# Accenture/AmpliGraph

Hardware: NVIDIA B200
Metric: training triples/sec (pos+eta negs) (higher is better)
Workload: dtype f32

## Files before the change

### ampligraph_b200/_lib.py

```python
import ctypes as C
import os
import subprocess

_HERE = os.path.dirname(os.path.abspath(__file__))
SO_PATH = os.environ.get("KGE_B200_LIB") or os.path.join(_HERE, "libkge_b200.so")
CSRC = os.path.join(_HERE, "csrc")
HEADER = os.path.join(os.path.dirname(_HERE), "include", "kge_b200.h")

KGE_OK, KGE_ERR_INVALID_ARGUMENT, KGE_ERR_CUDA, KGE_ERR_UNSUPPORTED = 0, 1, 2, 3
SCORING = {"TransE": 0, "DistMult": 1, "ComplEx": 2, "HolE": 3, "RotatE": 4}
LOSSES = {"pairwise": 0, "nll": 1, "absolute_margin": 2, "self_adversarial": 3, "multiclass_nll": 4}
REDUCTIONS = {"sum": 0, "mean": 1}
OPTIMIZERS = {"sgd": 0, "adam": 1, "adagrad": 2}
SIDES = {"s": 0, "o": 1}
STRATEGIES = {"worst": 0, "best": 1, "middle": 2}
STEP_FUSED, STEP_FORWARD_ONLY, STEP_BACKWARD_EXT = 0, 1, 2
RANK_MODES = {"auto": 0, "exact": 1}
INIT_KINDS = {"uniform": 0, "normal": 1, "truncated_normal": 2, "constant": 3}
ABI_VERSION = 2


class KgeConfig(C.Structure):
    _fields_ = [("struct_size", C.c_int32), ("scoring", C.c_int32), ("k", C.c_int32), ("eta", C.c_int32),
                ("n_ent", C.c_int64), ("n_rel", C.c_int64), ("loss", C.c_int32), ("reduction", C.c_int32),
                ("margin", C.c_float), ("alpha", C.c_float), ("device", C.c_int32), ("neg_group", C.c_int32),
                ("max_rel_size", C.c_int64), ("rank_mode", C.c_int32), ("rank_pair_cap", C.c_int32)]


class KgeOptimizerConfig(C.Structure):
    _fields_ = [("struct_size", C.c_int32), ("kind", C.c_int32), ("learning_rate", C.c_float),
                ("beta_1", C.c_float), ("beta_2", C.c_float), ("epsilon", C.c_float), ("momentum", C.c_float),
                ("initial_accumulator_value", C.c_float), ("reg_p", C.c_int32), ("reg_lambda", C.c_float),
                ("reg_p2", C.c_int32), ("reg_lambda2", C.c_float)]


class KgeShardMap(C.Structure):
    _fields_ = [("struct_size", C.c_int32), ("world", C.c_int32), ("rows_per_shard", C.c_int64),
                ("ent", C.c_void_p * 8), ("grad_ent", C.c_void_p * 8), ("stamp_ent", C.c_void_p * 8)]


_P = C.c_void_p
PROTOTYPES = {
    "kge_last_error": (C.c_char_p, []),
    "kge_abi_version": (C.c_int, []),
    "kge_create": (C.c_int, [C.POINTER(KgeConfig), C.POINTER(_P)]),
    "kge_destroy": (None, [_P]),
    "kge_internal_k": (C.c_int32, [_P]),
    "kge_half_stride": (C.c_int32, [_P]),
    "kge_row_stride": (C.c_int32, [_P]),
    "kge_pack_rows": (C.c_int, [_P, _P, _P, C.c_int64, _P]),
    "kge_unpack_rows": (C.c_int, [_P, _P, _P, C.c_int64, _P]),
    "kge_init_glorot_uniform": (C.c_int, [_P, _P, C.c_int64, C.c_uint64, _P]),
    "kge_init_table": (C.c_int, [_P, _P, C.c_int64, C.c_int32, C.c_float, C.c_float, C.c_uint64, _P]),
    "kge_score_triples": (C.c_int, [_P, _P, _P, _P, C.c_int64, _P, _P]),
    "kge_generate_corruptions": (C.c_int, [_P, _P, C.c_int64, C.c_uint64, C.c_uint64, _P, _P]),
    "kge_philox4x32_10": (None, [_P, _P, _P]),
    "kge_host_corruptions": (C.c_int, [_P, C.c_int64, C.c_int32, C.c_int64, C.c_uint64, C.c_uint64, _P]),
    "kge_train_step": (C.c_int, [_P, C.c_int32, _P, _P, _P, _P, _P, C.c_int64, _P, _P, C.c_uint64, C.c_uint64,
                                 _P, _P, _P, _P, _P, _P]),
    "kge_train_step_sharded": (C.c_int, [_P, C.c_int32, C.POINTER(KgeShardMap), _P, _P, _P, C.c_int64, _P, _P,
                                         C.c_uint64, C.c_uint64, _P, _P, _P, _P, _P, _P]),
    "kge_rank_sharded": (C.c_int, [_P, C.POINTER(KgeShardMap), C.c_int32, C.c_int32, C.c_int32, _P, _P, C.c_int64,
                                   _P, _P, C.c_int64, _P, _P, _P, C.c_int64, _P]),
    "kge_optimizer_step": (C.c_int, [_P, C.POINTER(KgeOptimizerConfig), C.c_int64, _P, _P, _P, _P, C.c_int64,
                                     _P, _P]),
    "kge_set_row_stamps": (C.c_int, [_P, _P, _P]),
    "kge_set_row_stash": (C.c_int, [_P, _P, C.c_int64]),
    "kge_set_hot_entities": (C.c_int, [_P, _P, C.c_int32]),
    "kge_rows_resident": (C.c_int, [_P]),
    "kge_step_stamp": (C.c_int32, [C.c_uint64]),
    "kge_optimizer_step_lazy": (C.c_int, [_P, C.POINTER(KgeOptimizerConfig), C.c_int64, _P, _P, _P, _P, C.c_int64, _P,
                                          C.c_int32, _P, _P]),
    "kge_optimizer_step_sharded": (C.c_int, [_P, C.POINTER(KgeOptimizerConfig), C.c_int64, C.c_int32, C.c_int32,
                                             C.POINTER(_P), C.POINTER(_P), _P, _P, C.c_int64, C.c_int64, _P, _P]),
    "kge_optimizer_step_exchange": (C.c_int, [_P, C.POINTER(KgeOptimizerConfig), C.POINTER(KgeOptimizerConfig), C.c_int64,
                                              C.c_int32, C.c_int32, C.POINTER(_P), C.POINTER(_P), _P, _P, _P, _P, _P,
                                              C.c_int64, C.c_int64, C.POINTER(_P), C.c_uint32, C.c_int32, _P, _P]),
    "kge_set_exchange_trace": (C.c_int, [_P, _P]),
    "kge_peer_barrier": (C.c_int, [_P, C.c_int32, C.c_int32, C.POINTER(_P), C.c_int32, C.c_uint32, _P]),
    "kge_rank": (C.c_int, [_P, C.c_int32, C.c_int32, _P, _P, _P, C.c_int64, _P, C.c_int64, C.c_int64, _P, _P,
                           C.c_int64, _P, _P, _P, C.c_int64, _P]),
    "kge_rank_finalize": (C.c_int, [_P, _P, C.c_int64, C.c_int32, _P, _P]),
    "kge_corruption_scores": (C.c_int, [_P, C.c_int32, _P, _P, _P, C.c_int64, _P, C.c_int64, C.c_int64, _P, _P,
                                        C.c_int64, _P]),
    "kge_rank_filter_probe": (C.c_int, [_P, C.c_int32, _P, _P, _P, C.c_int64, _P, C.c_int64, C.c_int64, _P, _P, _P,
                                        C.c_int64, _P]),
    "kge_rank_workspace_bytes": (C.c_int64, [_P, C.c_int64, C.c_int64]),
}

_lib = None


def build(verbose=False):
    cmd = ["make", "-C", CSRC, "-j8"]
    out = subprocess.run(cmd, stdout=subprocess.PIPE, stderr=subprocess.STDOUT, text=True)
    if verbose or out.returncode != 0:
        print(out.stdout)
    if out.returncode != 0:
        raise RuntimeError("building libkge_b200.so failed (see output above)")
    return SO_PATH


def load():
    global _lib
    if _lib is not None:
        return _lib
    if not os.path.exists(SO_PATH):
        raise RuntimeError(
            "ampligraph_b200: %s not found. Build it with `python -c 'import __graft_entry__ as g; g.build()'` "
            "or `make -C ampligraph_b200/csrc`. There is no CPU fallback for the CUDA path." % SO_PATH)
    lib = C.CDLL(SO_PATH)
    for name, (res, args) in PROTOTYPES.items():
        fn = getattr(lib, name)
        fn.restype = res
        fn.argtypes = args
    if lib.kge_abi_version() != ABI_VERSION:
        raise RuntimeError("libkge_b200.so ABI version %d, binding expects %d" % (lib.kge_abi_version(), ABI_VERSION))
    _lib = lib
    return lib


def check(rc):
# ... 19 lines not shown
```

### ampligraph_b200/csrc/kge_api.cu

```cuda
#include <stdarg.h>
#include <stdio.h>
#include <stdlib.h>
#include <string.h>

#include <new>

#include "kge_internal.h"

using namespace kge;

struct kge_handle {
    kge_config cfg;
    Layout L;
    int sm_count;
    int max_smem;
    float score_scale;
    float rot_div;
    float *rot;
    unsigned *done_counter;
    unsigned long long *exchange_trace;
    int nit, G, nbuf, warps, eta_pad, rows_bytes, region_bytes, wk, n_cb, slot_floats, resident;
    int res_warps, res_rows_bytes, res_region_bytes;
    int rot_warps, rot_G, rot_rows_bytes, rot_region_bytes;
    int *stamp_ent, *stamp_rel;
// ... 89 lines not shown
    Layout &L = h->L;
    L.model = cfg->scoring;
    L.k = cfg->k;
    L.halves = model_halves(cfg->scoring);
    L.kp = (cfg->k + 3) / 4 * 4;
    L.ld = L.halves * L.kp;
    L.K = L.halves * cfg->k;
    h->sm_count = prop.multiProcessorCount;
    h->max_smem = (int)prop.sharedMemPerBlockOptin;
    h->l2_bytes = prop.l2CacheSize;
    h->score_scale = (cfg->scoring == KGE_HOLE) ? hole_scale(L.K) : 1.f;
    h->rot_div = (cfg->scoring == KGE_ROTATE) ? rotate_divisor(L.K, cfg->max_rel_size > 0 ? cfg->max_rel_size : cfg->n_rel) : 1.f;

    const int nch = L.kp / 4;
    const int nit_raw = (nch + 31) / 32;
    h->nit = nit_raw <= 1 ? 1 : nit_raw <= 2 ? 2 : 4;
    h->wk = L.kp <= 512 ? L.kp : 512;
    h->n_cb = (L.kp + h->wk - 1) / h->wk;
    h->eta_pad = (cfg->eta + 3) / 4 * 4;
    const int row_bytes = L.halves * h->wk * 4, aux = 4 * h->eta_pad * 4 + 16;
    h->slot_floats = row_bytes / 4;
    int max_warps = KGE_TRAIN_THREADS(cfg->scoring, h->nit) / 32;
    int nbuf = 2;
    if (const char *ev = getenv("KGE_B200_TRAIN_WARPS")) { const int w = atoi(ev); if (w >= 1 && w < max_warps) max_warps = w; }
    if (const char *ev = getenv("KGE_B200_TRAIN_NBUF")) nbuf = atoi(ev) == 1 ? 1 : 2;
    int G = cfg->eta;
    bool res = h->n_cb == 1;
    if (cfg->neg_group > 0) {
        G = cfg->neg_group < cfg->eta ? cfg->neg_group : cfg->eta;
        res = res && G >= cfg->eta;
    } else {
        const long long full = (3 + (long long)cfg->eta) * row_bytes + aux;
        const int min_res = max_warps < KGE_MIN_RESIDENT_WARPS ? max_warps : KGE_MIN_RESIDENT_WARPS;
        if (!res || full * min_res > h->max_smem) {
            res = false;
            const int want = max_warps < KGE_TARGET_WARPS ? max_warps : KGE_TARGET_WARPS;
            while (G > 1 && (long long)((3 + nbuf * G) * (long long)row_bytes + aux) * want > h->max_smem) --G;
        }
    }
    h->resident = res ? 1 : 0;
    h->G = G;
    h->nbuf = nbuf;
    h->rows_bytes = (res ? 3 + G : 3 + nbuf * G) * row_bytes;
    h->region_bytes = h->rows_bytes + aux;
    int warps = h->max_smem / h->region_bytes;
    if (warps > max_warps) warps = max_warps;
    h->warps = warps;
    h->hot_ent[0] = h->hot_ent[1] = -1;

    h->res_warps = 0;
    if ((cfg->scoring == KGE_DISTMULT || cfg->scoring == KGE_COMPLEX || cfg->scoring == KGE_HOLE) && h->n_cb == 1 &&
        (h->nit <= 2 || cfg->scoring == KGE_DISTMULT) && cfg->eta <= 32 && cfg->neg_group <= 0) {
        const int res_aux = (3 * h->eta_pad * 4 + 8 + 15) / 16 * 16;
        h->res_rows_bytes = (2 + cfg->eta) * row_bytes;
        h->res_region_bytes = h->res_rows_bytes + res_aux;
        int rw = h->max_smem / h->res_region_bytes;
        if (rw > max_warps) rw = max_warps;
        int min_res = max_warps < KGE_MIN_RESIDENT_WARPS ? max_warps : KGE_MIN_RESIDENT_WARPS;
        if (h->nit == 4) min_res = KGE_MIN_RESIDENT_WARPS_WIDE;
        if (const char *ev = getenv("KGE_B200_RES_MIN_WARPS")) min_res = atoi(ev);
        if (rw >= min_res) h->res_warps = rw;
    }

    h->rot_warps = 0;
    if (cfg->scoring == KGE_ROTATE && h->n_cb == 1 && h->nit <= 2 && cfg->neg_group <= 0) {
        const int rot_aux = (4 * h->eta_pad * 4 + 16 + 15) / 16 * 16;
        const int rw = 8;
        const int cap = (h->max_smem / rw - rot_aux) / row_bytes;
        int rG = cap >= cfg->eta ? cfg->eta : cap / 2;
        if (const char *ev = getenv("KGE_B200_ROT_G")) {
            const int g = atoi(ev);
            if (g >= 1 && g <= cap / 2 && g < cfg->eta) rG = g;
        }
        if (rG >= 1) {
            h->rot_warps = rw;
            h->rot_G = rG;
            h->rot_rows_bytes = (rG >= cfg->eta ? rG : 2 * rG) * row_bytes;
            h->rot_region_bytes = h->rot_rows_bytes + rot_aux;
        }
    }

    if (cfg->scoring == KGE_ROTATE) {
        cudaError_t e2 = cudaMalloc(&h->rot, (size_t)cfg->n_rel * L.ld * sizeof(float));
        if (e2 != cudaSuccess) { delete h; return cuda_fail(e2, "cudaMalloc(rotation table)"); }
    }
    {
        cudaError_t e2 = cudaMalloc(&h->done_counter, 4 * sizeof(unsigned));
        if (e2 == cudaSuccess) e2 = cudaMemset(h->done_counter, 0, 4 * sizeof(unsigned));
        if (e2 != cudaSuccess) { if (h->rot) cudaFree(h->rot); delete h; return cuda_fail(e2, "cudaMalloc(counter)"); }
    }
    *out = h;
    return KGE_OK;
}

extern "C" void kge_destroy(kge_handle *h)
{
    if (!h) return;
    DeviceGuard guard_(h->cfg.device);
    if (h->rot) cudaFree(h->rot);
    if (h->done_counter) cudaFree(h->done_counter);
    delete h;
}

extern "C" int32_t kge_internal_k(const kge_handle *h) { return h ? h->L.K : 0; }
extern "C" int32_t kge_half_stride(const kge_handle *h) { return h ? h->L.kp : 0; }
extern "C" int32_t kge_row_stride(const kge_handle *h) { return h ? h->L.ld : 0; }

#define KGE_CHECK_HANDLE(h, fn)                                           \
    if (!(h)) return fail(KGE_ERR_INVALID_ARGUMENT, fn ": null handle"); \
    KGE_GUARD(h)

// ... 261 lines not shown
static RegParams reg_of(const kge_optimizer_config *opt)
{
    RegParams r;
    r.p = opt->reg_p; r.lambda = opt->reg_lambda; r.p2 = opt->reg_p2; r.lambda2 = opt->reg_lambda2;
    return r;
}
static void fill_optim(const kge_optimizer_config *opt, int64_t t, OptimParams &o)
{
    o.kind = opt->kind;
    o.lr = opt->learning_rate;
    o.beta1 = opt->beta_1;
    o.beta2 = opt->beta_2;
    o.eps = opt->epsilon;
    o.momentum = opt->momentum;
    o.reg = reg_of(opt);
    o.lr_t = (float)((double)opt->learning_rate * sqrt(1.0 - pow((double)opt->beta_2, (double)t)) /
                     (1.0 - pow((double)opt->beta_1, (double)t)));
}
static bool slots_ok(const kge_optimizer_config *opt, const float *s0, const float *s1)
{
    const bool need0 = opt->kind != KGE_OPT_SGD || opt->momentum != 0.f;
    const bool need1 = opt->kind == KGE_OPT_ADAM;
    return !((need0 && !s0) || (need1 && !s1));
}

extern "C" int kge_optimizer_step(kge_handle *h, const kge_optimizer_config *opt, int64_t t, float *table_dev,
                                  float *grad_dev, float *slot0_dev, float *slot1_dev, int64_t rows,
                                  double *reg_loss_dev, void *stream)
{
    KGE_CHECK_HANDLE(h, "kge_optimizer_step");
    if (int rc = check_optim(opt, "kge_optimizer_step")) return rc;
    if (rows < 0 || t < 1) return fail(KGE_ERR_INVALID_ARGUMENT, "kge_optimizer_step: rows >= 0 and t >= 1 required");
    if (rows == 0) return KGE_OK;
    if (!table_dev || !grad_dev) return fail(KGE_ERR_INVALID_ARGUMENT, "kge_optimizer_step: null table/grad");
    if (!slots_ok(opt, slot0_dev, slot1_dev))
        return fail(KGE_ERR_INVALID_ARGUMENT, "kge_optimizer_step: optimizer slot buffer missing");
    OptimParams o;
    fill_optim(opt, t, o);
    KGE_CUDA(launch_optimizer(o, table_dev, grad_dev, slot0_dev, slot1_dev, rows * (long long)h->L.ld, reg_loss_dev,
                              h->sm_count, (cudaStream_t)stream),
             "kge_optimizer_step");
    return KGE_OK;
}

extern "C" int kge_set_row_stamps(kge_handle *h, int32_t *ent_stamps_dev, int32_t *rel_stamps_dev)
{
    KGE_CHECK_HANDLE(h, "kge_set_row_stamps");
    h->stamp_ent = ent_stamps_dev;
    h->stamp_rel = rel_stamps_dev;
    return KGE_OK;
}

extern "C" int kge_rows_resident(const kge_handle *h) { return h ? (h->resident ? 1 : 0) : -1; }

extern "C" int kge_set_hot_entities(kge_handle *h, const int32_t *ids_host, int32_t n)
{
    KGE_CHECK_HANDLE(h, "kge_set_hot_entities");
    if (n < 0 || (n > 0 && !ids_host)) return fail(KGE_ERR_INVALID_ARGUMENT, "kge_set_hot_entities: bad arguments");
    h->hot_ent[0] = h->hot_ent[1] = -1;
    for (int i = 0; i < n && i < 2; ++i) {
        if (ids_host[i] < 0 || ids_host[i] >= h->cfg.n_ent) return fail(KGE_ERR_INVALID_ARGUMENT, "kge_set_hot_entities: id %d out of range", ids_host[i]);
        if (i == 1 && ids_host[1] == ids_host[0]) break;
        h->hot_ent[i] = ids_host[i];
    }
    return KGE_OK;
}

extern "C" int kge_set_row_stash(kge_handle *h, float *stash_dev, int64_t rows)
{
    KGE_CHECK_HANDLE(h, "kge_set_row_stash");
    if (rows < 0) return fail(KGE_ERR_INVALID_ARGUMENT, "kge_set_row_stash: rows < 0");
    h->stash = stash_dev;
    h->stash_rows = stash_dev ? rows : 0;
    return KGE_OK;
}

extern "C" int32_t kge_step_stamp(uint64_t step) { return (int32_t)(step & 0x3fffffffu) + 1; }

extern "C" int kge_optimizer_step_lazy(kge_handle *h, const kge_optimizer_config *opt, int64_t t, float *table_dev,
                                       float *grad_dev, float *slot0_dev, float *slot1_dev, int64_t rows,
                                       const int32_t *row_stamp_dev, int32_t stamp, double *reg_loss_dev, void *stream)
{
    KGE_CHECK_HANDLE(h, "kge_optimizer_step_lazy");
    if (int rc = check_optim(opt, "kge_optimizer_step_lazy")) return rc;
    if (rows < 0 || t < 1) return fail(KGE_ERR_INVALID_ARGUMENT, "kge_optimizer_step_lazy: rows >= 0 and t >= 1 required");
    if (rows == 0) return KGE_OK;
    if (!table_dev || !grad_dev || !row_stamp_dev) return fail(KGE_ERR_INVALID_ARGUMENT, "kge_optimizer_step_lazy: null pointer");
    if (!slots_ok(opt, slot0_dev, slot1_dev))
        return fail(KGE_ERR_INVALID_ARGUMENT, "kge_optimizer_step_lazy: optimizer slot buffer missing");
    OptimParams o;
    fill_optim(opt, t, o);
    KGE_CUDA(launch_optimizer_lazy(o, table_dev, grad_dev, slot0_dev, slot1_dev, rows, h->L.ld, (const int *)row_stamp_dev,
                                   stamp, reg_loss_dev, h->sm_count, (cudaStream_t)stream),
             "kge_optimizer_step_lazy");
    return KGE_OK;
}

static int check_world(int32_t world, int32_t rank, const char *fn)
{
    if (world < 1 || world > KGE_MAX_PEERS || rank < 0 || rank >= world)
        return fail(KGE_ERR_INVALID_ARGUMENT, "%s: world must be 1..%d and 0 <= rank < world", fn, KGE_MAX_PEERS);
    return KGE_OK;
}

extern "C" int kge_optimizer_step_sharded(kge_handle *h, const kge_optimizer_config *opt, int64_t t, int32_t world,
                                          int32_t rank, float *const *peer_tables, float *const *peer_grads,
// ... 265 lines not shown
```

### ampligraph_b200/csrc/kge_internal.h

```cpp
#pragma once
#include "kge_common.cuh"

#define KGE_TRAIN_THREADS(model, nit) ((nit) <= 1 ? 512 : (nit) == 2 ? ((model) == KGE_ROTATE ? 256 : 384) : 256)
#define KGE_MAX_PEERS 8
#define KGE_MIN_RESIDENT_WARPS 8
#define KGE_TARGET_WARPS 10
#define KGE_MIN_RESIDENT_WARPS_WIDE 6

namespace kge {

struct TrainParams {
    const float *ent;
    const float *rel;
    float *grad_ent;
    float *grad_rel;
    const int32_t *triples;
    long long B;
    const int32_t *neg_ent;
    const uint8_t *neg_keep;
    unsigned long long seed, step;
    unsigned n_ent;
    int model, eta, kp, ld, nch;
    int G;
    int nbuf;
    int wk, n_cb;
    int slot_floats;
    int resident;
    int eta_pad;
    int rows_bytes, region_bytes;
    int loss, reduction, mode;
    float margin, alpha, score_scale, inv_div;
    double *loss_out;
    float *scores_pos, *scores_neg;
    const float *dpos, *dneg;
    int shard_world, rows_per_shard;
    const float *ent_shard[KGE_MAX_PEERS];
    float *grad_ent_shard[KGE_MAX_PEERS];
    int stamp;
    int *stamp_ent, *stamp_rel;
    int *stamp_ent_shard[KGE_MAX_PEERS];
    int hot_ent[2];
    float *stash;
    unsigned *sched;
};

cudaError_t launch_train(const TrainParams &p, int nit, int sm_count, int threads, size_t smem, cudaStream_t st);
cudaError_t launch_train_res(const TrainParams &p, int nit, int sm_count, int threads, size_t smem, cudaStream_t st);
cudaError_t launch_train_rot(const TrainParams &p, int nit, int sm_count, int threads, size_t smem, cudaStream_t st);
cudaError_t launch_rotation_table(const float *rel, float *rot, long long n_rel, int kp, int ld, float div,
                                  cudaStream_t st);
cudaError_t launch_corruptions(const int32_t *triples, long long B, int eta, unsigned long long seed,
                               unsigned long long step, unsigned n_ent, int32_t *out, cudaStream_t st);

cudaError_t launch_score_triples(const Layout &L, int nit, const float *ent, const float *rel_or_rot,
                                 const int32_t *triples, long long n, float scale, float *out, int sm_count,
                                 cudaStream_t st);
// ... 83 lines not shown
```

### ampligraph_b200/csrc/kge_train_res.cu

```cuda
#include "kge_train_common.cuh"

namespace kge {

#ifndef KGE_HOT
#define KGE_HOT 1
#endif

template <int HALVES, int NIT, int THREADS>
__global__ void __launch_bounds__(THREADS) kge_train_res_kernel(const TrainParams p)
{
    extern __shared__ __align__(128) unsigned char smem_raw[];
    int warp = threadIdx.x >> 5, lane = threadIdx.x & 31;
    KGE_KEEP32(warp);
    KGE_KEEP32(lane);
    uint32_t rows_s = smem_u32(smem_raw) + (uint32_t)warp * (uint32_t)p.region_bytes;
    uint32_t sc_s = rows_s + (uint32_t)p.rows_bytes;
    uint32_t nid_s = sc_s + 4u * (uint32_t)p.eta_pad;
    uint32_t jor_s = nid_s + 4u * (uint32_t)p.eta_pad;
    uint32_t bar_s = jor_s + 4u * (uint32_t)p.eta_pad;
    KGE_KEEP32(rows_s); KGE_KEEP32(sc_s); KGE_KEEP32(nid_s); KGE_KEEP32(jor_s); KGE_KEEP32(bar_s);
    float *const sc = reinterpret_cast<float *>(smem_raw + (size_t)warp * p.region_bytes + p.rows_bytes);

    if (lane == 0) mbar_init_s(bar_s, 1);
    fence_mbar_init();
    fence_proxy_async_smem();
    __syncthreads();

    int ld = p.ld, eta = p.eta;
    const int nch = p.kp >> 2;
    uint32_t lwB = (uint32_t)p.slot_floats * 4u;
    uint32_t hsB = (uint32_t)p.kp * 4u;
    uint32_t row_bytes = (uint32_t)ld * 4u;
    KGE_KEEP32(ld); KGE_KEEP32(eta); KGE_KEEP32(lwB); KGE_KEEP32(hsB); KGE_KEEP32(row_bytes);
    uint32_t off[NIT];
    int live_i[NIT];
#pragma unroll
    for (int it = 0; it < NIT; ++it) {
        const int c = lane + 32 * it;
        live_i[it] = c < nch ? 1 : 0;
        off[it] = 16u * (uint32_t)min(c, nch - 1);
        KGE_KEEP32(off[it]);
        KGE_KEEP32(live_i[it]);
    }
    bool live[NIT];
#pragma unroll
    for (int it = 0; it < NIT; ++it) live[it] = live_i[it] != 0;
    float scale = p.score_scale;
    KGE_KEEPF(scale);
    unsigned lt = (1u << lane) - 1u;
    KGE_KEEP32(lt);
    float *grad_ent = p.grad_ent;
    KGE_KEEP64(grad_ent);
    const bool stamping = p.stamp_ent != nullptr && p.mode != KGE_STEP_FORWARD_ONLY;
    uint32_t phase = 0u;
    double loss_acc = 0.0;
    int hot0 = p.hot_ent[0], hot1 = KGE_HOT > 1 ? p.hot_ent[1] : -1;
    KGE_KEEP32(hot0); KGE_KEEP32(hot1);
    float4 H0r[NIT], H0i[NIT], H1r[NIT], H1i[NIT];
#pragma unroll
    for (int it = 0; it < NIT; ++it) H0r[it] = H0i[it] = H1r[it] = H1i[it] = f4zero();

    const long long n_warps = (long long)gridDim.x * (blockDim.x >> 5);
    float next_draw = 0.f;
    for (long long i = (long long)blockIdx.x * (blockDim.x >> 5) + warp; i < p.B;
         i = p.sched ? n_warps + (long long)(unsigned)__shfl_sync(0xffffffffu, next_draw, 0) : i + n_warps) {
        if (p.sched && lane == 0) next_draw = sched_draw(p.sched);
        int tv = 0;
        if (lane < 3) tv = __ldg(p.triples + 3 * i + lane);
        const int s_id = __shfl_sync(0xffffffffu, tv, 0), p_id = __shfl_sync(0xffffffffu, tv, 1), o_id = __shfl_sync(0xffffffffu, tv, 2);
        int keep = -1, repl = 0;
        if (lane < eta) {
            const unsigned long long r = (unsigned long long)lane * (unsigned long long)p.B + (unsigned long long)i;
            if (p.neg_ent) { repl = p.neg_ent[r]; keep = p.neg_keep[r] ? 1 : 0; }
            else draw_corruption(p.seed, p.step, r, p.n_ent, &keep, &repl);
        }
        const unsigned m0 = __ballot_sync(0xffffffffu, keep == 0), m1 = __ballot_sync(0xffffffffu, keep == 1);
        const int n0 = __popc(m0);
        if (lane < eta) {
            const int t = keep ? n0 + __popc(m1 & lt) : __popc(m0 & lt);
            sts_i(nid_s + 4u * (uint32_t)t, repl);
            sts_i(jor_s + 4u * (uint32_t)t, lane);
            if (stamping) p.stamp_ent[repl] = p.stamp;
        }
        if (stamping) {
            if (lane == 0) p.stamp_ent[s_id] = p.stamp;
            if (lane == 1) p.stamp_ent[o_id] = p.stamp;
            if (lane == 2 && p.stamp_rel) p.stamp_rel[p_id] = p.stamp;
        }
        __syncwarp();

        const int nrow = 2 + eta;
        if (lane == 0) mbar_expect_tx_s(bar_s, (uint32_t)nrow * row_bytes);
        __syncwarp();
        for (int r = lane; r < nrow; r += 32) {
            const int id = r == 0 ? s_id : r == 1 ? o_id : lds_i(nid_s + 4u * (uint32_t)(r - 2));
            bulk_load_s(rows_s + (uint32_t)r * lwB, p.ent + (size_t)id * ld, row_bytes, bar_s);
        }
        float4 pr[NIT], pi[NIT];
        {
            const char *prow = reinterpret_cast<const char *>(p.rel + (size_t)p_id * ld);
#pragma unroll
            for (int it = 0; it < NIT; ++it) {
                pr[it] = __ldg(reinterpret_cast<const float4 *>(prow + off[it]));
                if constexpr (HALVES == 2) pi[it] = __ldg(reinterpret_cast<const float4 *>(prow + off[it] + hsB));
                if (!live[it]) { pr[it] = f4zero(); pi[it] = f4zero(); }
            }
        }
        char *const gs_row = reinterpret_cast<char *>(grad_ent + (size_t)s_id * ld);
        char *const gp_row = reinterpret_cast<char *>(p.grad_rel + (size_t)p_id * ld);
        char *const go_row = reinterpret_cast<char *>(grad_ent + (size_t)o_id * ld);
        mbar_wait_s(bar_s, phase);
        phase ^= 1u;

        float4 Q0r[NIT], Q0i[NIT], Q1r[NIT], Q1i[NIT];
        float4 W0r[NIT], W0i[NIT], W1r[NIT], W1i[NIT];
        float P;
        {
            float4 acc = f4zero();
#pragma unroll
            for (int it = 0; it < NIT; ++it) {
                const uint32_t a = rows_s + off[it];
                if constexpr (HALVES == 2) {
                    const float4 sr = lds4(a), si = lds4(a + hsB);
                    const float4 orr = lds4(a + lwB), oi = lds4(a + lwB + hsB);
                    Q0r[it] = f4fma(pi[it], oi, pr[it] * orr);
                    Q0i[it] = pr[it] * oi - pi[it] * orr;
                    Q1r[it] = sr * pr[it] - si * pi[it];
                    Q1i[it] = f4fma(sr, pi[it], si * pr[it]);
                    acc = f4fma(sr, Q0r[it], acc);
                    acc = f4fma(si, Q0i[it], acc);
                    W0i[it] = W1i[it] = f4zero();
                } else {
                    const float4 vs = lds4(a), vo = lds4(a + lwB);
                    Q0r[it] = pr[it] * vo;
                    Q1r[it] = vs * pr[it];
                    acc = f4fma(vs, Q0r[it], acc);
                }
                W0r[it] = W1r[it] = f4zero();
            }
            P = warp_sum(f4hsum(acc));
        }

        auto score_side = [&](int lo, int hi, const float4(&qr)[NIT], const float4(&qi)[NIT]) {
            int t = lo;
            for (; hi - t >= 3; t += 4) {
                const uint32_t r0 = rows_s + (uint32_t)(2 + t) * lwB, r1 = r0 + lwB, r2 = r1 + lwB;
                const uint32_t r3 = (t + 3 < hi) ? r2 + lwB : r2;
                float4 a = f4zero(), b = f4zero(), c = f4zero(), d = f4zero();
#pragma unroll
                for (int it = 0; it < NIT; ++it) {
                    const uint32_t o = off[it];
                    a = f4fma(lds4(r0 + o), qr[it], a);
                    b = f4fma(lds4(r1 + o), qr[it], b);
                    c = f4fma(lds4(r2 + o), qr[it], c);
                    d = f4fma(lds4(r3 + o), qr[it], d);
                    if constexpr (HALVES == 2) {
                        a = f4fma(lds4(r0 + o + hsB), qi[it], a);
                        b = f4fma(lds4(r1 + o + hsB), qi[it], b);
                        c = f4fma(lds4(r2 + o + hsB), qi[it], c);
                        d = f4fma(lds4(r3 + o + hsB), qi[it], d);
                    }
                }
                const float v = warp_sum4t(f4hsum(a), f4hsum(b), f4hsum(c), f4hsum(d), lane);
                const int q = lane >> 3;
                if ((lane & 7) == 0 && t + q < hi) sts_f(sc_s + 4u * (uint32_t)(t + q), v);
            }
            if (t < hi) {
                const bool has_b = t + 1 < hi;
                const uint32_t ra = rows_s + (uint32_t)(2 + t) * lwB, rb = has_b ? ra + lwB : ra;
                float4 a = f4zero(), b = f4zero();
#pragma unroll
                for (int it = 0; it < NIT; ++it) {
                    const uint32_t o = off[it];
                    a = f4fma(lds4(ra + o), qr[it], a);
                    b = f4fma(lds4(rb + o), qr[it], b);
                    if constexpr (HALVES == 2) {
                        a = f4fma(lds4(ra + o + hsB), qi[it], a);
                        b = f4fma(lds4(rb + o + hsB), qi[it], b);
                    }
                }
                float pa = f4hsum(a), pb = f4hsum(b);
                warp_sum2(pa, pb);
                if (lane == 0) {
                    sts_f(sc_s + 4u * (uint32_t)t, pa);
                    if (has_b) sts_f(sc_s + 4u * (uint32_t)(t + 1), pb);
                }
            }
        };
        score_side(0, n0, Q0r, Q0i);
        score_side(n0, eta, Q1r, Q1i);
        __syncwarp();

        float dP;
        if (p.mode != KGE_STEP_BACKWARD_EXT) {
            if (scale != 1.f) {
                if (lane < eta) sc[lane] *= scale;
                __syncwarp();
            }
            if (p.scores_neg && lane < eta) p.scores_neg[(size_t)lds_i(jor_s + 4u * (uint32_t)lane) * p.B + i] = sc[lane];
            if (p.scores_pos && lane == 0) p.scores_pos[i] = scale * P;
            if (p.mode == KGE_STEP_FORWARD_ONLY) { __syncwarp(); continue; }
            const float li = loss_and_dscores(p, scale * P, sc, lane, &dP);
            if (lane == 0) loss_acc += (double)li;
        } else {
            if (lane < eta) sc[lane] = p.dneg[(size_t)lds_i(jor_s + 4u * (uint32_t)lane) * p.B + i];
            dP = p.dpos[i];
        }
        __syncwarp();

        auto red_row = [&](int id, float g, const float4(&qr)[NIT], const float4(&qi)[NIT]) {
            if (!live[0]) return;
            char *const g0 = reinterpret_cast<char *>(grad_ent + (size_t)id * ld) + off[0];
            char *const g1 = g0 + hsB;
#pragma unroll
            for (int it = 0; it < NIT; ++it) {
                if (!live[it]) break;
                red_add_v4(reinterpret_cast<float *>(g0 + 512 * it), g * qr[it]);
                if constexpr (HALVES == 2) red_add_v4(reinterpret_cast<float *>(g1 + 512 * it), g * qi[it]);
            }
        };
        auto grad_side = [&](int lo, int hi, const float4(&qr)[NIT], const float4(&qi)[NIT], float4(&Wr)[NIT], float4(&Wi)[NIT]) {
            for (int t = lo; t < hi; t += 2) {
                const bool has_b = t + 1 < hi;
                const uint32_t tb = (uint32_t)(has_b ? t + 1 : t);
                const uint32_t ra = rows_s + (uint32_t)(2 + t) * lwB, rb = rows_s + (2u + tb) * lwB;
                const float ga = scale * lds_f(sc_s + 4u * (uint32_t)t);
                const float gb = has_b ? scale * lds_f(sc_s + 4u * tb) : 0.f;
                const int ida = lds_i(nid_s + 4u * (uint32_t)t), idb = lds_i(nid_s + 4u * tb);
#pragma unroll
                for (int it = 0; it < NIT; ++it) {
                    const uint32_t o = off[it];
                    const float4 ar = lds4(ra + o), br = lds4(rb + o);
                    Wr[it] = f4fma(ga, ar, Wr[it]);
                    Wr[it] = f4fma(gb, br, Wr[it]);
                    if constexpr (HALVES == 2) {
                        const float4 ai = lds4(ra + o + hsB), bi = lds4(rb + o + hsB);
                        Wi[it] = f4fma(ga, ai, Wi[it]);
                        Wi[it] = f4fma(gb, bi, Wi[it]);
                    }
                }
                red_row(ida, ga, qr, qi);
                if (has_b) red_row(idb, gb, qr, qi);
            }
        };
        grad_side(0, n0, Q0r, Q0i, W0r, W0i);
        grad_side(n0, eta, Q1r, Q1i, W1r, W1i);

        {
            const float gP = scale * dP;
#pragma unroll
            for (int it = 0; it < NIT; ++it) {
                if (!live[it]) continue;
                const uint32_t o = off[it], a = rows_s + o;
                if constexpr (HALVES == 2) {
                    const float4 sr = lds4(a), si = lds4(a + hsB);
                    const float4 orr = lds4(a + lwB), oi = lds4(a + lwB + hsB);
                    const float4 Ur = f4fma(gP, sr, W0r[it]), Ui = f4fma(gP, si, W0i[it]);
                    const float4 Xr = f4fma(gP, orr, W1r[it]), Xi = f4fma(gP, oi, W1i[it]);
                    const float4 gsr = f4fma(pi[it], Xi, pr[it] * Xr), gsi = pr[it] * Xi - pi[it] * Xr;
                    const float4 gor = Ur * pr[it] - Ui * pi[it], goi = f4fma(Ur, pi[it], Ui * pr[it]);
                    if (s_id == hot0) { H0r[it] = H0r[it] + gsr; H0i[it] = H0i[it] + gsi; }
                    else if (KGE_HOT > 1 && s_id == hot1) { H1r[it] = H1r[it] + gsr; H1i[it] = H1i[it] + gsi; }
                    else { red4(gs_row, o, gsr); red4(gs_row, o + hsB, gsi); }
                    if (o_id == hot0) { H0r[it] = H0r[it] + gor; H0i[it] = H0i[it] + goi; }
                    else if (KGE_HOT > 1 && o_id == hot1) { H1r[it] = H1r[it] + gor; H1i[it] = H1i[it] + goi; }
                    else { red4(go_row, o, gor); red4(go_row, o + hsB, goi); }
                    red4(gp_row, o, f4fma(Ur, orr, Ui * oi) + f4fma(sr, W1r[it], si * W1i[it]));
                    red4(gp_row, o + hsB, (Ur * oi - Ui * orr) + (sr * W1i[it] - si * W1r[it]));
                } else {
                    const float4 vs = lds4(a), vo = lds4(a + lwB);
                    const float4 U = f4fma(gP, vs, W0r[it]), X = f4fma(gP, vo, W1r[it]);
                    const float4 gsr = pr[it] * X, gor = U * pr[it];
                    if (s_id == hot0) H0r[it] = H0r[it] + gsr;
                    else if (KGE_HOT > 1 && s_id == hot1) H1r[it] = H1r[it] + gsr;
                    else red4(gs_row, o, gsr);
                    if (o_id == hot0) H0r[it] = H0r[it] + gor;
                    else if (KGE_HOT > 1 && o_id == hot1) H1r[it] = H1r[it] + gor;
                    else red4(go_row, o, gor);
                    red4(gp_row, o, f4fma(U, vo, vs * W1r[it]));
                }
            }
        }
        __syncwarp();
    }
    sched_retire(p.sched, n_warps, lane);
    if (p.mode != KGE_STEP_FORWARD_ONLY) {
#pragma unroll
        for (int h = 0; h < KGE_HOT; ++h) {
            const int id = h ? hot1 : hot0;
            if (id < 0) continue;
            char *const row = reinterpret_cast<char *>(grad_ent + (size_t)id * ld);
#pragma unroll
            for (int it = 0; it < NIT; ++it) {
                if (!live[it]) continue;
                red4(row, off[it], h ? H1r[it] : H0r[it]);
                if constexpr (HALVES == 2) red4(row, off[it] + hsB, h ? H1i[it] : H0i[it]);
            }
        }
    }
    if (p.loss_out && p.mode == KGE_STEP_FUSED && lane == 0 && loss_acc != 0.0) atomicAdd(p.loss_out, loss_acc);
}

template <int HALVES, int NIT>
static cudaError_t launch_res(const TrainParams &p, int sm_count, int threads, size_t smem, cudaStream_t st)
{
    constexpr int THREADS = KGE_TRAIN_THREADS(KGE_COMPLEX, NIT);
    auto kern = kge_train_res_kernel<HALVES, NIT, THREADS>;
    cudaError_t e = cudaFuncSetAttribute(kern, cudaFuncAttributeMaxDynamicSharedMemorySize, (int)smem);
    if (e != cudaSuccess) return e;
    int occ = 0;
    e = cudaOccupancyMaxActiveBlocksPerMultiprocessor(&occ, kern, threads, smem);
    if (e != cudaSuccess) return e;
    if (occ < 1) return cudaErrorLaunchOutOfResources;
    const long long want = (p.B + (threads / 32) - 1) / (threads / 32), cap = (long long)occ * sm_count;
    kern<<<(int)(want < cap ? want : cap), threads, smem, st>>>(p);
    return cudaGetLastError();
}

cudaError_t launch_train_res(const TrainParams &p, int nit, int sm_count, int threads, size_t smem, cudaStream_t st)
{
    if (p.B == 0) return cudaSuccess;
    const bool two = p.model != KGE_DISTMULT;
    if (nit <= 1) return two ? launch_res<2, 1>(p, sm_count, threads, smem, st) : launch_res<1, 1>(p, sm_count, threads, smem, st);
    if (nit == 2) return two ? launch_res<2, 2>(p, sm_count, threads, smem, st) : launch_res<1, 2>(p, sm_count, threads, smem, st);
    if (two) return cudaErrorInvalidValue;
    return launch_res<1, 4>(p, sm_count, threads, smem, st);
}

}
```

### include/kge_b200.h

```cpp
#ifndef KGE_B200_H
#define KGE_B200_H

#include <stdint.h>

#ifdef __cplusplus
extern "C" {
#endif

#define KGE_B200_ABI_VERSION 2

typedef struct kge_handle kge_handle;

enum kge_status {
    KGE_OK = 0,
    KGE_ERR_INVALID_ARGUMENT = 1,
    KGE_ERR_CUDA = 2,
    KGE_ERR_UNSUPPORTED = 3
};

enum kge_scoring { KGE_TRANSE = 0, KGE_DISTMULT = 1, KGE_COMPLEX = 2, KGE_HOLE = 3, KGE_ROTATE = 4 };

enum kge_loss {
    KGE_LOSS_PAIRWISE = 0,
    KGE_LOSS_NLL = 1,
// ... 47 lines not shown
    int32_t reg_p;
    float reg_lambda;
    int32_t reg_p2;
    float reg_lambda2;
} kge_optimizer_config;

const char *kge_last_error(void);
int kge_abi_version(void);

int kge_create(const kge_config *cfg, kge_handle **out);
void kge_destroy(kge_handle *h);

int32_t kge_internal_k(const kge_handle *h);
int32_t kge_half_stride(const kge_handle *h);
int32_t kge_row_stride(const kge_handle *h);

int kge_pack_rows(kge_handle *h, const float *dense_dev, float *table_dev, int64_t rows, void *stream);
int kge_unpack_rows(kge_handle *h, const float *table_dev, float *dense_dev, int64_t rows, void *stream);

int kge_init_glorot_uniform(kge_handle *h, float *table_dev, int64_t rows, uint64_t seed, void *stream);
int kge_init_table(kge_handle *h, float *table_dev, int64_t rows, int32_t kind, float a, float b, uint64_t seed,
                   void *stream);

int kge_score_triples(kge_handle *h, const float *ent_dev, const float *rel_dev,
                      const int32_t *triples_dev , int64_t n, float *scores_dev ,
                      void *stream);

int kge_generate_corruptions(kge_handle *h, const int32_t *triples_dev, int64_t B, uint64_t seed,
                             uint64_t step, int32_t *corruptions_dev , void *stream);

void kge_philox4x32_10(const uint32_t ctr[4], const uint32_t key[2], uint32_t out[4]);
int kge_host_corruptions(const int32_t *triples_host , int64_t B, int32_t eta, int64_t n_ent,
                         uint64_t seed, uint64_t step, int32_t *corruptions_host );

int kge_train_step(kge_handle *h, int32_t mode, const float *ent_dev, const float *rel_dev,
                   float *grad_ent_dev, float *grad_rel_dev, const int32_t *triples_dev, int64_t B,
                   const int32_t *neg_ent_dev, const uint8_t *neg_keep_subj_dev, uint64_t seed,
                   uint64_t step, double *loss_dev, float *scores_pos_dev, float *scores_neg_dev,
                   const float *dpos_dev, const float *dneg_dev, void *stream);

typedef struct kge_shard_map {
    int32_t struct_size;
    int32_t world;
    int64_t rows_per_shard;
    const float *ent[8];
    float *grad_ent[8];
    int32_t *stamp_ent[8];
} kge_shard_map;

int kge_set_row_stash(kge_handle *h, float *stash_dev, int64_t rows);

int kge_set_hot_entities(kge_handle *h, const int32_t *ids_host, int32_t n);
int kge_rows_resident(const kge_handle *h);

int kge_train_step_sharded(kge_handle *h, int32_t mode, const kge_shard_map *map, const float *rel_dev,
                           float *grad_rel_dev, const int32_t *triples_dev, int64_t B,
                           const int32_t *neg_ent_dev, const uint8_t *neg_keep_subj_dev, uint64_t seed,
                           uint64_t step, double *loss_dev, float *scores_pos_dev, float *scores_neg_dev,
                           const float *dpos_dev, const float *dneg_dev, void *stream);

int kge_optimizer_step(kge_handle *h, const kge_optimizer_config *opt, int64_t t, float *table_dev,
                       float *grad_dev, float *slot0_dev, float *slot1_dev, int64_t rows,
                       double *reg_loss_dev, void *stream);

int kge_set_row_stamps(kge_handle *h, int32_t *ent_stamps_dev, int32_t *rel_stamps_dev);
int32_t kge_step_stamp(uint64_t step);
int kge_optimizer_step_lazy(kge_handle *h, const kge_optimizer_config *opt, int64_t t, float *table_dev,
                            float *grad_dev, float *slot0_dev, float *slot1_dev, int64_t rows,
                            const int32_t *row_stamp_dev, int32_t stamp, double *reg_loss_dev, void *stream);

int kge_optimizer_step_sharded(kge_handle *h, const kge_optimizer_config *opt, int64_t t, int32_t world,
                               int32_t rank, float *const *peer_tables, float *const *peer_grads,
                               float *slot0_shard_dev, float *slot1_shard_dev, int64_t row_begin,
                               int64_t row_end, double *reg_loss_dev, void *stream);

int kge_optimizer_step_exchange(kge_handle *h, const kge_optimizer_config *opt_ent,
                                const kge_optimizer_config *opt_rel, int64_t t, int32_t world, int32_t rank,
                                float *const *peer_tables, float *const *peer_grads, float *table_mc_dev,
                                const float *grads_mc_dev, float *zero_grads_dev,
                                float *slot0_shard_dev, float *slot1_shard_dev, int64_t row_begin,
                                int64_t row_end, uint32_t *const *peer_flags, uint32_t token, int32_t phases,
                                double *reg_loss_dev, void *stream);

int kge_set_exchange_trace(kge_handle *h, uint64_t *stamps_dev);

int kge_peer_barrier(kge_handle *h, int32_t world, int32_t rank, uint32_t *const *peer_flags, int32_t slot,
                     uint32_t token, void *stream);

int kge_rank(kge_handle *h, int32_t side, int32_t strategy, const float *ent_dev,
             const float *rel_dev, const int32_t *triples_dev, int64_t b,
             const int32_t *cand_ids_dev, int64_t cand_begin, int64_t n_cand,
             const int64_t *filt_off_dev, const int32_t *filt_idx_dev, int64_t n_filt,
             int32_t *ranks_dev, int32_t *counts_dev, void *workspace_dev, int64_t workspace_bytes,
             void *stream);

int kge_rank_sharded(kge_handle *h, const kge_shard_map *map, int32_t rank, int32_t side, int32_t strategy,
                     const float *rel_dev, const int32_t *triples_dev, int64_t b,
                     const int64_t *filt_off_dev, const int32_t *filt_idx_dev, int64_t n_filt,
                     int32_t *ranks_dev, int32_t *counts_dev, void *workspace_dev, int64_t workspace_bytes,
                     void *stream);

int kge_rank_finalize(kge_handle *h, const int32_t *counts_dev , int64_t b, int32_t strategy,
                      int32_t *ranks_dev, void *stream);

int kge_corruption_scores(kge_handle *h, int32_t side, const float *ent_dev, const float *rel_dev,
                          const int32_t *triples_dev, int64_t b, const int32_t *cand_ids_dev,
// ... 15 lines not shown
```

Baseline: 1.824 billion.

## Load s/o rows to registers, shrink smem region, add hot-free kernel variant

```diff
diff --git a/ampligraph_b200/_lib.py b/ampligraph_b200/_lib.py
--- a/ampligraph_b200/_lib.py
+++ b/ampligraph_b200/_lib.py
@@ -68,6 +68,7 @@
     "kge_set_row_stash": (C.c_int, [_P, _P, C.c_int64]),
     "kge_set_hot_entities": (C.c_int, [_P, _P, C.c_int32]),
     "kge_rows_resident": (C.c_int, [_P]),
+    "kge_train_fast_warps": (C.c_int, [_P]),
     "kge_step_stamp": (C.c_int32, [C.c_uint64]),
     "kge_optimizer_step_lazy": (C.c_int, [_P, C.POINTER(KgeOptimizerConfig), C.c_int64, _P, _P, _P, _P, C.c_int64, _P,
                                           C.c_int32, _P, _P]),
diff --git a/ampligraph_b200/csrc/kge_api.cu b/ampligraph_b200/csrc/kge_api.cu
--- a/ampligraph_b200/csrc/kge_api.cu
+++ b/ampligraph_b200/csrc/kge_api.cu
@@ -165,11 +165,13 @@
     if ((cfg->scoring == KGE_DISTMULT || cfg->scoring == KGE_COMPLEX || cfg->scoring == KGE_HOLE) && h->n_cb == 1 &&
         (h->nit <= 2 || cfg->scoring == KGE_DISTMULT) && cfg->eta <= 32 && cfg->neg_group <= 0) {
         const int res_aux = (3 * h->eta_pad * 4 + 8 + 15) / 16 * 16;
-        h->res_rows_bytes = (2 + cfg->eta) * row_bytes;
+        h->res_rows_bytes = cfg->eta * row_bytes;
         h->res_region_bytes = h->res_rows_bytes + res_aux;
+        int res_max = KGE_RES_THREADS(h->nit) / 32;
+        if (const char *ev = getenv("KGE_B200_TRAIN_WARPS")) { const int w = atoi(ev); if (w >= 1 && w < res_max) res_max = w; }
         int rw = h->max_smem / h->res_region_bytes;
-        if (rw > max_warps) rw = max_warps;
-        int min_res = max_warps < KGE_MIN_RESIDENT_WARPS ? max_warps : KGE_MIN_RESIDENT_WARPS;
+        if (rw > res_max) rw = res_max;
+        int min_res = res_max < KGE_MIN_RESIDENT_WARPS ? res_max : KGE_MIN_RESIDENT_WARPS;
         if (h->nit == 4) min_res = KGE_MIN_RESIDENT_WARPS_WIDE;
         if (const char *ev = getenv("KGE_B200_RES_MIN_WARPS")) min_res = atoi(ev);
         if (rw >= min_res) h->res_warps = rw;
@@ -537,6 +539,7 @@
 }
 
 extern "C" int kge_rows_resident(const kge_handle *h) { return h ? (h->resident ? 1 : 0) : -1; }
+extern "C" int kge_train_fast_warps(const kge_handle *h) { return h ? h->res_warps : -1; }
 
 extern "C" int kge_set_hot_entities(kge_handle *h, const int32_t *ids_host, int32_t n)
 {
diff --git a/ampligraph_b200/csrc/kge_internal.h b/ampligraph_b200/csrc/kge_internal.h
--- a/ampligraph_b200/csrc/kge_internal.h
+++ b/ampligraph_b200/csrc/kge_internal.h
@@ -2,6 +2,7 @@
 #include "kge_common.cuh"
 
 #define KGE_TRAIN_THREADS(model, nit) ((nit) <= 1 ? 512 : (nit) == 2 ? ((model) == KGE_ROTATE ? 256 : 384) : 256)
+#define KGE_RES_THREADS(nit) ((nit) <= 1 ? 512 : (nit) == 2 ? 448 : 256)
 #define KGE_MAX_PEERS 8
 #define KGE_MIN_RESIDENT_WARPS 8
 #define KGE_TARGET_WARPS 10
diff --git a/ampligraph_b200/csrc/kge_train_res.cu b/ampligraph_b200/csrc/kge_train_res.cu
--- a/ampligraph_b200/csrc/kge_train_res.cu
+++ b/ampligraph_b200/csrc/kge_train_res.cu
@@ -1,12 +1,19 @@
 #include "kge_train_common.cuh"
 
 namespace kge {
+
+__device__ __forceinline__ float4 ldg4_nc(const char *p)
+{
+    float4 v;
+    asm volatile("ld.global.nc.v4.f32 {%0, %1, %2, %3}, [%4];" : "=f"(v.x), "=f"(v.y), "=f"(v.z), "=f"(v.w) : "l"(p));
+    return v;
+}
 
 #ifndef KGE_HOT
 #define KGE_HOT 1
 #endif
 
-template <int HALVES, int NIT, int THREADS>
+template <int HALVES, int NIT, int THREADS, bool HOT>
 __global__ void __launch_bounds__(THREADS) kge_train_res_kernel(const TrainParams p)
 {
     extern __shared__ __align__(128) unsigned char smem_raw[];
@@ -89,28 +96,31 @@
         }
         __syncwarp();
 
-        const int nrow = 2 + eta;
-        if (lane == 0) mbar_expect_tx_s(bar_s, (uint32_t)nrow * row_bytes);
-        __syncwarp();
-        for (int r = lane; r < nrow; r += 32) {
-            const int id = r == 0 ? s_id : r == 1 ? o_id : lds_i(nid_s + 4u * (uint32_t)(r - 2));
-            bulk_load_s(rows_s + (uint32_t)r * lwB, p.ent + (size_t)id * ld, row_bytes, bar_s);
-        }
+        if (lane == 0) mbar_expect_tx_s(bar_s, (uint32_t)eta * row_bytes);
+        __syncwarp();
+        if (lane < eta) bulk_load_s(rows_s + (uint32_t)lane * lwB, p.ent + (size_t)lds_i(nid_s + 4u * (uint32_t)lane) * ld, row_bytes, bar_s);
         float4 pr[NIT], pi[NIT];
+        float4 sr[NIT], si[NIT], orr[NIT], oi[NIT];
         {
+            const char *const s_src = reinterpret_cast<const char *>(p.ent + (size_t)s_id * ld);
+            const char *const o_src = reinterpret_cast<const char *>(p.ent + (size_t)o_id * ld);
             const char *prow = reinterpret_cast<const char *>(p.rel + (size_t)p_id * ld);
 #pragma unroll
             for (int it = 0; it < NIT; ++it) {
+                sr[it] = __ldg(reinterpret_cast<const float4 *>(s_src + off[it]));
+                orr[it] = __ldg(reinterpret_cast<const float4 *>(o_src + off[it]));
                 pr[it] = __ldg(reinterpret_cast<const float4 *>(prow + off[it]));
-                if constexpr (HALVES == 2) pi[it] = __ldg(reinterpret_cast<const float4 *>(prow + off[it] + hsB));
+                if constexpr (HALVES == 2) {
+                    si[it] = __ldg(reinterpret_cast<const float4 *>(s_src + off[it] + hsB));
+                    oi[it] = __ldg(reinterpret_cast<const float4 *>(o_src + off[it] + hsB));
+                    pi[it] = __ldg(reinterpret_cast<const float4 *>(prow + off[it] + hsB));
+                }
                 if (!live[it]) { pr[it] = f4zero(); pi[it] = f4zero(); }
             }
         }
         char *const gs_row = reinterpret_cast<char *>(grad_ent + (size_t)s_id * ld);
         char *const gp_row = reinterpret_cast<char *>(p.grad_rel + (size_t)p_id * ld);
         char *const go_row = reinterpret_cast<char *>(grad_ent + (size_t)o_id * ld);
-        mbar_wait_s(bar_s, phase);
-        phase ^= 1u;
 
         float4 Q0r[NIT], Q0i[NIT], Q1r[NIT], Q1i[NIT];
         float4 W0r[NIT], W0i[NIT], W1r[NIT], W1i[NIT];
@@ -119,32 +129,30 @@
             float4 acc = f4zero();
 #pragma unroll
             for (int it = 0; it < NIT; ++it) {
-                const uint32_t a = rows_s + off[it];
-                if constexpr (HALVES == 2) {
-                    const float4 sr = lds4(a), si = lds4(a + hsB);
-                    const float4 orr = lds4(a + lwB), oi = lds4(a + lwB + hsB);
-                    Q0r[it] = f4fma(pi[it], oi, pr[it] * orr);
-                    Q0i[it] = pr[it] * oi - pi[it] * orr;
-                    Q1r[it] = sr * pr[it] - si * pi[it];
-                    Q1i[it] = f4fma(sr, pi[it], si * pr[it]);
-                    acc = f4fma(sr, Q0r[it], acc);
-                    acc = f4fma(si, Q0i[it], acc);
+                if constexpr (HALVES == 2) {
+                    Q0r[it] = f4fma(pi[it], oi[it], pr[it] * orr[it]);
+                    Q0i[it] = pr[it] * oi[it] - pi[it] * orr[it];
+                    Q1r[it] = sr[it] * pr[it] - si[it] * pi[it];
+                    Q1i[it] = f4fma(sr[it], pi[it], si[it] * pr[it]);
+                    acc = f4fma(sr[it], Q0r[it], acc);
+                    acc = f4fma(si[it], Q0i[it], acc);
                     W0i[it] = W1i[it] = f4zero();
                 } else {
-                    const float4 vs = lds4(a), vo = lds4(a + lwB);
-                    Q0r[it] = pr[it] * vo;
-                    Q1r[it] = vs * pr[it];
-                    acc = f4fma(vs, Q0r[it], acc);
+                    Q0r[it] = pr[it] * orr[it];
+                    Q1r[it] = sr[it] * pr[it];
+                    acc = f4fma(sr[it], Q0r[it], acc);
                 }
                 W0r[it] = W1r[it] = f4zero();
             }
             P = warp_sum(f4hsum(acc));
         }
+        mbar_wait_s(bar_s, phase);
+        phase ^= 1u;
 
         auto score_side = [&](int lo, int hi, const float4(&qr)[NIT], const float4(&qi)[NIT]) {
             int t = lo;
             for (; hi - t >= 3; t += 4) {
-                const uint32_t r0 = rows_s + (uint32_t)(2 + t) * lwB, r1 = r0 + lwB, r2 = r1 + lwB;
+                const uint32_t r0 = rows_s + (uint32_t)t * lwB, r1 = r0 + lwB, r2 = r1 + lwB;
                 const uint32_t r3 = (t + 3 < hi) ? r2 + lwB : r2;
                 float4 a = f4zero(), b = f4zero(), c = f4zero(), d = f4zero();
 #pragma unroll
@@ -167,7 +175,7 @@
             }
             if (t < hi) {
                 const bool has_b = t + 1 < hi;
-                const uint32_t ra = rows_s + (uint32_t)(2 + t) * lwB, rb = has_b ? ra + lwB : ra;
+                const uint32_t ra = rows_s + (uint32_t)t * lwB, rb = has_b ? ra + lwB : ra;
                 float4 a = f4zero(), b = f4zero();
 #pragma unroll
                 for (int it = 0; it < NIT; ++it) {
@@ -223,7 +231,7 @@
             for (int t = lo; t < hi; t += 2) {
                 const bool has_b = t + 1 < hi;
                 const uint32_t tb = (uint32_t)(has_b ? t + 1 : t);
-                const uint32_t ra = rows_s + (uint32_t)(2 + t) * lwB, rb = rows_s + (2u + tb) * lwB;
+                const uint32_t ra = rows_s + (uint32_t)t * lwB, rb = rows_s + tb * lwB;
                 const float ga = scale * lds_f(sc_s + 4u * (uint32_t)t);
                 const float gb = has_b ? scale * lds_f(sc_s + 4u * tb) : 0.f;
                 const int ida = lds_i(nid_s + 4u * (uint32_t)t), idb = lds_i(nid_s + 4u * tb);
@@ -243,39 +251,64 @@
                 if (has_b) red_row(idb, gb, qr, qi);
             }
         };
+#if KGE_RES_PREFETCH
+        {
+            const long long ent_off = reinterpret_cast<const char *>(p.ent) - reinterpret_cast<const char *>(grad_ent);
+#pragma unroll
+            for (int it = 0; it < NIT; ++it) {
+                asm volatile("prefetch.global.L1 [%0];" ::"l"(gs_row + ent_off + off[it]));
+                asm volatile("prefetch.global.L1 [%0];" ::"l"(go_row + ent_off + off[it]));
+                if constexpr (HALVES == 2) {
+                    asm volatile("prefetch.global.L1 [%0];" ::"l"(gs_row + ent_off + off[it] + hsB));
+                    asm volatile("prefetch.global.L1 [%0];" ::"l"(go_row + ent_off + off[it] + hsB));
+                }
+            }
+        }
+#endif
         grad_side(0, n0, Q0r, Q0i, W0r, W0i);
         grad_side(n0, eta, Q1r, Q1i, W1r, W1i);
 
         {
             const float gP = scale * dP;
+            const long long ent_off = reinterpret_cast<const char *>(p.ent) - reinterpret_cast<const char *>(grad_ent);
+            const char *const s_src = gs_row + ent_off, *const o_src = go_row + ent_off;
+            float4 vsr[NIT], vsi[NIT], vor[NIT], voi[NIT];
+#pragma unroll
+            for (int it = 0; it < NIT; ++it) {
+                vsr[it] = ldg4_nc(s_src + off[it]);
+                vor[it] = ldg4_nc(o_src + off[it]);
+                if constexpr (HALVES == 2) {
+                    vsi[it] = ldg4_nc(s_src + off[it] + hsB);
+                    voi[it] = ldg4_nc(o_src + off[it] + hsB);
+                }
+            }
 #pragma unroll
             for (int it = 0; it < NIT; ++it) {
                 if (!live[it]) continue;
-                const uint32_t o = off[it], a = rows_s + o;
-                if constexpr (HALVES == 2) {
-                    const float4 sr = lds4(a), si = lds4(a + hsB);
-                    const float4 orr = lds4(a + lwB), oi = lds4(a + lwB + hsB);
+                const uint32_t o = off[it];
+                if constexpr (HALVES == 2) {
+                    const float4 sr = vsr[it], si = vsi[it], orr = vor[it], oi = voi[it];
                     const float4 Ur = f4fma(gP, sr, W0r[it]), Ui = f4fma(gP, si, W0i[it]);
                     const float4 Xr = f4fma(gP, orr, W1r[it]), Xi = f4fma(gP, oi, W1i[it]);
                     const float4 gsr = f4fma(pi[it], Xi, pr[it] * Xr), gsi = pr[it] * Xi - pi[it] * Xr;
                     const float4 gor = Ur * pr[it] - Ui * pi[it], goi = f4fma(Ur, pi[it], Ui * pr[it]);
-                    if (s_id == hot0) { H0r[it] = H0r[it] + gsr; H0i[it] = H0i[it] + gsi; }
-                    else if (KGE_HOT > 1 && s_id == hot1) { H1r[it] = H1r[it] + gsr; H1i[it] = H1i[it] + gsi; }
+                    if (HOT && s_id == hot0) { H0r[it] = H0r[it] + gsr; H0i[it] = H0i[it] + gsi; }
+                    else if (HOT && KGE_HOT > 1 && s_id == hot1) { H1r[it] = H1r[it] + gsr; H1i[it] = H1i[it] + gsi; }
                     else { red4(gs_row, o, gsr); red4(gs_row, o + hsB, gsi); }
-                    if (o_id == hot0) { H0r[it] = H0r[it] + gor; H0i[it] = H0i[it] + goi; }
-                    else if (KGE_HOT > 1 && o_id == hot1) { H1r[it] = H1r[it] + gor; H1i[it] = H1i[it] + goi; }
+                    if (HOT && o_id == hot0) { H0r[it] = H0r[it] + gor; H0i[it] = H0i[it] + goi; }
+                    else if (HOT && KGE_HOT > 1 && o_id == hot1) { H1r[it] = H1r[it] + gor; H1i[it] = H1i[it] + goi; }
                     else { red4(go_row, o, gor); red4(go_row, o + hsB, goi); }
                     red4(gp_row, o, f4fma(Ur, orr, Ui * oi) + f4fma(sr, W1r[it], si * W1i[it]));
                     red4(gp_row, o + hsB, (Ur * oi - Ui * orr) + (sr * W1i[it] - si * W1r[it]));
                 } else {
-                    const float4 vs = lds4(a), vo = lds4(a + lwB);
+                    const float4 vs = vsr[it], vo = vor[it];
                     const float4 U = f4fma(gP, vs, W0r[it]), X = f4fma(gP, vo, W1r[it]);
                     const float4 gsr = pr[it] * X, gor = U * pr[it];
-                    if (s_id == hot0) H0r[it] = H0r[it] + gsr;
-                    else if (KGE_HOT > 1 && s_id == hot1) H1r[it] = H1r[it] + gsr;
+                    if (HOT && s_id == hot0) H0r[it] = H0r[it] + gsr;
+                    else if (HOT && KGE_HOT > 1 && s_id == hot1) H1r[it] = H1r[it] + gsr;
                     else red4(gs_row, o, gsr);
-                    if (o_id == hot0) H0r[it] = H0r[it] + gor;
-                    else if (KGE_HOT > 1 && o_id == hot1) H1r[it] = H1r[it] + gor;
+                    if (HOT && o_id == hot0) H0r[it] = H0r[it] + gor;
+                    else if (HOT && KGE_HOT > 1 && o_id == hot1) H1r[it] = H1r[it] + gor;
                     else red4(go_row, o, gor);
                     red4(gp_row, o, f4fma(U, vo, vs * W1r[it]));
                 }
@@ -284,7 +317,7 @@
         __syncwarp();
     }
     sched_retire(p.sched, n_warps, lane);
-    if (p.mode != KGE_STEP_FORWARD_ONLY) {
+    if (HOT && p.mode != KGE_STEP_FORWARD_ONLY) {
 #pragma unroll
         for (int h = 0; h < KGE_HOT; ++h) {
             const int id = h ? hot1 : hot0;
@@ -304,8 +337,9 @@
 template <int HALVES, int NIT>
 static cudaError_t launch_res(const TrainParams &p, int sm_count, int threads, size_t smem, cudaStream_t st)
 {
-    constexpr int THREADS = KGE_TRAIN_THREADS(KGE_COMPLEX, NIT);
-    auto kern = kge_train_res_kernel<HALVES, NIT, THREADS>;
+    constexpr int THREADS = KGE_RES_THREADS(NIT);
+    const bool hot = p.hot_ent[0] >= 0 || (KGE_HOT > 1 && p.hot_ent[1] >= 0);
+    auto kern = hot ? kge_train_res_kernel<HALVES, NIT, THREADS, true> : kge_train_res_kernel<HALVES, NIT, THREADS, false>;
     cudaError_t e = cudaFuncSetAttribute(kern, cudaFuncAttributeMaxDynamicSharedMemorySize, (int)smem);
     if (e != cudaSuccess) return e;
     int occ = 0;
diff --git a/include/kge_b200.h b/include/kge_b200.h
--- a/include/kge_b200.h
+++ b/include/kge_b200.h
@@ -123,6 +123,7 @@
 
 int kge_set_hot_entities(kge_handle *h, const int32_t *ids_host, int32_t n);
 int kge_rows_resident(const kge_handle *h);
+int kge_train_fast_warps(const kge_handle *h);
 
 int kge_train_step_sharded(kge_handle *h, int32_t mode, const kge_shard_map *map, const float *rel_dev,
                            float *grad_rel_dev, const int32_t *triples_dev, int64_t B,
```

New measurement: 1.841 billion (median of 6 runs). Within noise of the previous version (+0.9%).
